# scalable-arch/CAL_22-MPC

Measured on AMD Instinct MI355X. Metric: 64B blocks/s (whole node) + achieved HBM GB/s fraction; ratio bit-exact vs CPU, higher is better.
Workload: dtype u8; 1 GPU; 268435456 random_u32 64 B blocks per GPU, VPC probe config (6 modules, all predictors); algorithm=VPC, line_size=64, blocks_per_gpu=268435456

## Files before the change

cal_22-mpc_amd/csrc/mpc_ring.h:

```cpp
#pragma once
#include "mpc_kernel_common.h"

#ifndef MPC_RING_NT
#define MPC_RING_NT 1
#endif

template <int NQ>
__device__ __forceinline__ u32 ring_swz(u32 line) { return (line >> (NQ == 2 ? 3 : (NQ == 4 ? 2 : 1))) & (u32)(NQ - 1); }

template <int NQ>
__device__ __forceinline__ u32 ring_src_off(int j, u32 lane)
{
  const u32 q = 64u * (u32)j + lane, line = q / NQ, pos = q % NQ;
  return 16u * (line * NQ + (pos ^ ring_swz<NQ>(line))) - 1024u * (u32)j;
}

template <int NQ>
__device__ __forceinline__ u32 ring_rd_off(u32 ll, int k) { return 16u * (ll * NQ + ((u32)k ^ ring_swz<NQ>(ll))); }

#if MPC_RING_NT
#define MPC_GLDS_AUX " nt"
#else
#define MPC_GLDS_AUX ""
#endif
template <int NP>
__device__ __forceinline__ void ring_glds(const u32 *lane_off, const void *gbase, u32 lds_dst)
{
  u32 keep;
  if constexpr (NP == 4)
    asm volatile("s_mov_b32 %0, m0\n\ts_mov_b32 m0, %6\n\ts_nop 0\n\t"
                 "global_load_lds_dwordx4 %1, %5" MPC_GLDS_AUX "\n\tglobal_load_lds_dwordx4 %2, %5 offset:1024" MPC_GLDS_AUX "\n\t"
                 "global_load_lds_dwordx4 %3, %5 offset:2048" MPC_GLDS_AUX "\n\tglobal_load_lds_dwordx4 %4, %5 offset:3072" MPC_GLDS_AUX "\n\t"
                 "s_mov_b32 m0, %0"
                 : "=&s"(keep) : "v"(lane_off[0]), "v"(lane_off[1]), "v"(lane_off[2]), "v"(lane_off[3]), "s"(gbase), "s"(lds_dst));
  else
    asm volatile("s_mov_b32 %0, m0\n\ts_mov_b32 m0, %4\n\ts_nop 0\n\t"
                 "global_load_lds_dwordx4 %1, %3" MPC_GLDS_AUX "\n\tglobal_load_lds_dwordx4 %2, %3 offset:1024" MPC_GLDS_AUX "\n\t"
                 "s_mov_b32 m0, %0"
                 : "=&s"(keep) : "v"(lane_off[0]), "v"(lane_off[1]), "s"(gbase), "s"(lds_dst));
}

template <int NQ>
__device__ __forceinline__ void ring_request(const u32 (&lane_off)[NQ], const uint4 *gbase_, u32 lds_dst_)
{
  const u64 gb = reinterpret_cast<u64>(gbase_);
  const u32 gb_hi = (u32)__builtin_amdgcn_readfirstlane((int)(u32)(gb >> 32)), gb_lo = (u32)__builtin_amdgcn_readfirstlane((int)(u32)gb);
  const uint4 *gbase = reinterpret_cast<const uint4 *>(((u64)gb_hi << 32) | (u64)gb_lo);
  const u32 lds_dst = (u32)__builtin_amdgcn_readfirstlane((int)lds_dst_);
  if constexpr (NQ == 8) {
    ring_glds<4>(&lane_off[0], gbase, lds_dst);
    ring_glds<4>(&lane_off[4], gbase + 256, lds_dst + 4096u);
  } else {
    ring_glds<NQ>(&lane_off[0], gbase, lds_dst);
  }
}

__device__ __forceinline__ u32 uni(u32 x) { return (u32)__builtin_amdgcn_readfirstlane((int)x); }
__device__ __forceinline__ bool uni(bool x) { return __builtin_amdgcn_readfirstlane((int)x) != 0; }

template <int N>
__device__ __forceinline__ void ring_wait_vm() { asm volatile("s_waitcnt vmcnt(%0)" ::"i"(N)); }

template <int NQ>
__device__ __forceinline__ void ring_read(uint4 (&v)[NQ], const u32 (&a)[NQ])
{
  typedef u32 v4 __attribute__((ext_vector_type(4)));
  v4 r[NQ];
  if constexpr (NQ == 2)
    asm volatile("ds_read_b128 %0, %2\n\tds_read_b128 %1, %3\n\ts_waitcnt lgkmcnt(0)"
                 : "=&v"(r[0]), "=&v"(r[1]) : "v"(a[0]), "v"(a[1]));
  else if constexpr (NQ == 4)
    asm volatile("ds_read_b128 %0, %4\n\tds_read_b128 %1, %5\n\tds_read_b128 %2, %6\n\tds_read_b128 %3, %7\n\ts_waitcnt lgkmcnt(0)"
                 : "=&v"(r[0]), "=&v"(r[1]), "=&v"(r[2]), "=&v"(r[3]) : "v"(a[0]), "v"(a[1]), "v"(a[2]), "v"(a[3]));
  else
    asm volatile("ds_read_b128 %0, %8\n\tds_read_b128 %1, %9\n\tds_read_b128 %2, %10\n\tds_read_b128 %3, %11\n\t"
                 "ds_read_b128 %4, %12\n\tds_read_b128 %5, %13\n\tds_read_b128 %6, %14\n\tds_read_b128 %7, %15\n\ts_waitcnt lgkmcnt(0)"
                 : "=&v"(r[0]), "=&v"(r[1]), "=&v"(r[2]), "=&v"(r[3]), "=&v"(r[4]), "=&v"(r[5]), "=&v"(r[6]), "=&v"(r[7])
                 : "v"(a[0]), "v"(a[1]), "v"(a[2]), "v"(a[3]), "v"(a[4]), "v"(a[5]), "v"(a[6]), "v"(a[7]));
#pragma unroll
  for (int k = 0; k < NQ; k++) v[k] = make_uint4(r[k].x, r[k].y, r[k].z, r[k].w);
}
```

cal_22-mpc_amd/csrc/mpc_vpc_lane.hip:

```cpp
#include "mpc_kernel_common.h"
#include "mpc_ring.h"

#ifndef MPC_JIT_BM
#define MPC_JIT_BM 0
#endif
#ifndef MPC_JIT_ANYROOT
#define MPC_JIT_ANYROOT 0
#endif
#ifndef MPC_JIT_PLANES
#define MPC_JIT_PLANES 0
#endif
#ifndef MPC_JIT_GATHER
#define MPC_JIT_GATHER 0
#endif
#ifndef MPC_JIT_WSHIFT
#define MPC_JIT_WSHIFT 0
#endif
#ifndef MPC_DRAIN_WAIT
#define MPC_DRAIN_WAIT 1
#endif
#ifndef MPC_CERT_TIERS
#define MPC_CERT_TIERS 1
#endif
#ifndef MPC_ABLATE
#define MPC_ABLATE 0
#endif
namespace {

constexpr int LK_PW = 8;
constexpr int LK_PW2 = 16;
__device__ __host__ constexpr int lk_base(int kind) { return kind & 7; }
__device__ __host__ constexpr int lk_dist(int kind) { return (kind & LK_PW2) ? 2 : ((kind & LK_PW) ? 1 : 0); }

typedef const u32 __attribute__((address_space(4))) *ctab_t;
__device__ __forceinline__ ctab_t lane_tab(const MpcVpcParams &P) { return (ctab_t)(u64)P.tab; }

#if MPC_JIT_ANYROOT || MPC_JIT_GATHER || MPC_JIT_WSHIFT
template <int Q>
__device__ __forceinline__ MpcFastModule lane_fm_const(const MpcVpcParams &P)
{
  MpcFastModule f = P.fm[Q];
#if MPC_JIT_ANYROOT
  constexpr int roots[] = {MPC_JIT_ROOTS};
  f.root = roots[Q];
#endif
#if MPC_JIT_GATHER
  constexpr int gathers[] = {MPC_JIT_GATHERS};
  f.gather = gathers[Q] ? Q + 1 : 0;
#endif
#if MPC_JIT_WSHIFT
  constexpr int wgens[] = {MPC_JIT_WGENS};
  f.wgen = wgens[Q] ? Q + 1 : 0;
#endif
  return f;
}
#define LANE_FM(Q) lane_fm_const<Q>(P)
#else
#define LANE_FM(Q) P.fm[Q]
#endif

template <int W>
struct Lane {
  u32 x[W];
  u32 b0;
  u32 rootb;
  bool gen;
  ctab_t trunc;
};

template <int W>
__device__ __forceinline__ u32 lane_root_bytes(const Lane<W> &c, int root)
{
  const int rw = root >> 2;
  u32 xw = 0;
#pragma unroll
  for (int e = 0; e < (MPC_JIT_ANYROOT ? W : 4); e++) xw = and_or(c.x[e], 0u - (u32)(e == rw), xw);
  return perm(xw, xw, 0x01010101u * (u32)(root & 3));
}
__device__ __forceinline__ u32 lane_onebase_pred(u32 rb, int root, int e)
{
  const u32 here = (e == (root >> 2)) ? (0xffu << (8 * (root & 3))) : 0u;
  return rb & ~here;
}
__device__ __forceinline__ u32 lane_row0_word(u32 msbs, int root, int e)
{
  return (MPC_JIT_ANYROOT && e == 3 && root > 15) ? (msbs & 0x00ffffffu) : msbs;
}
template <int W, int NR>
__device__ __forceinline__ void lane_root_to_front(const Lane<W> &c, int root, u32 (&r)[W])
{
  u32 prev = lane_root_bytes<W>(c, root) & 0xff000000u;
#pragma unroll
  for (int e = 0; e < (MPC_JIT_ANYROOT ? NR : (NR < 4 ? NR : 4)); e++) {
    const u32 sh = alignbyte(r[e], prev, 3);
    const int nb = root + 1 - 4 * e;
    const u32 m = nb >= 4 ? ~0u : (nb <= 0 ? 0u : ((1u << (8 * nb)) - 1u));
    prev = r[e];
    r[e] = mask_sel(m, sh, r[e]);
  }
}

__device__ __forceinline__ u32 msb_of_bsub(u32 a, u32 b) { return ((a | H80) - (b & L7F)) ^ a ^ ~b; }

template <int W>
__device__ __forceinline__ u32 plane_bytes(const u32 (&x)[W], int q, int k)
// ... 152 lines not shown
    if (MPC_JIT_ANYROOT && c.gen && E0 == 0 && fm.root > 15) m |= lane_root_bytes<W>(c, fm.root);
  }
  return m & H80;
}

template <int W>
__device__ __forceinline__ u32 lane_leading_zero_rows(const u32 (&r)[W], ctab_t scan_mask = nullptr, u32 plane_mask = ~0u)
{
  constexpr int NG = W / 4;
  u32 S[NG], G = 0;
  if (scan_mask) {
#pragma unroll
    for (int j = 0; j < NG; j++) {
      S[j] = (r[4 * j] & scan_mask[4 * j]) | (r[4 * j + 1] & scan_mask[4 * j + 1]) | (r[4 * j + 2] & scan_mask[4 * j + 2]) |
             (r[4 * j + 3] & scan_mask[4 * j + 3]);
      G |= S[j];
    }
  } else {
#pragma unroll
    for (int j = 0; j < NG; j++) {
      S[j] = r[4 * j] | r[4 * j + 1] | r[4 * j + 2] | r[4 * j + 3];
      G |= S[j];
    }
  }
  const u32 gf = fold8(G) & plane_mask;
  const u32 p = (u32)__clz((int)gf) - 24u;
  const u32 B = H80 >> (p & 7u);
  u32 j_star = NG - 1;
#pragma unroll
  for (int j = NG - 2; j >= 0; j--) j_star = (S[j] & B) ? (u32)j : j_star;
  return (plane_mask == ~0u ? G : gf) ? NG * p + j_star : 2u * W;
}

__device__ __forceinline__ bool lane_bit(u64 mask) { return __builtin_amdgcn_inverse_ballot_w64(mask); }

template <int W>
struct LaneBest {
  u32 r[W];
  u32 z;
  int q;
  u32 root_r;
  u32 cx;
  u32 pm;
  u32 encb;
};

#ifndef MPC_DEFER_MAX
#define MPC_DEFER_MAX 8
#endif

#ifndef MPC_PAIR_PROBE
#define MPC_PAIR_PROBE 64
#endif
constexpr u32 kPairProbe = MPC_PAIR_PROBE;

__host__ __device__ static inline size_t lane_stats_smem(int K, int bins)
{
  return 16 * (size_t)((2 * K * 8 + 15) / 16) + 16 * (size_t)(((K * bins + 2) * 4 + 15) / 16);
}

template <int W, int KIND>
__device__ __forceinline__ u32 lane_row0_bm(const Lane<W> &c, const MpcFastModule &fm, ctab_t tab)
{
  u32 r[W], root_r;
  lane_residue<W, KIND, 1>(c, fm, tab, r, root_r);
  return r[0] & (c.trunc ? (c.trunc[0] & 0xffffu) : 0xffffu);
}

template <int W, int NPT, int Q>
__device__ __forceinline__ u32 lane_row0_min(const Lane<W> &, const MpcVpcParams &) { return ~0u; }

template <int W, int NPT, int Q, int KIND, int... REST>
__device__ __forceinline__ u32 lane_row0_min(const Lane<W> &c, const MpcVpcParams &P)
{
  if constexpr (Q + 1 == NPT) {
    return ~0u;
  } else {
    const u32 m = MPC_JIT_BM ? lane_row0_bm<W, KIND>(c, LANE_FM(Q), lane_tab(P)) : lane_row0<W, KIND, 0, 3>(c, LANE_FM(Q), lane_tab(P));
    return min(m, lane_row0_min<W, NPT, Q + 1, REST...>(c, P));
  }
}

template <int W, int NPT, int Q>
__device__ __forceinline__ u32 lane_prefilters(const Lane<W> &, const MpcVpcParams &, u64 &, u64 &, bool, bool &) { return 0; }

template <int W, int NPT, int Q, int KIND, int... REST>
__device__ __forceinline__ u32 lane_prefilters(const Lane<W> &c, const MpcVpcParams &P, u64 &need_mask, u64 &defer_mask,
                                               bool allow_defer, bool &alt)
{
  if constexpr (Q + 1 == NPT) {
    return 0;
  } else {
    u32 bit = 0;
    if constexpr (!(MPC_ABLATE & 8)) {
      u32 msb = MPC_JIT_BM ? lane_row0_bm<W, KIND>(c, LANE_FM(Q), lane_tab(P)) : lane_row0<W, KIND, 0, 3>(c, LANE_FM(Q), lane_tab(P));
      if ((__ballot(msb != 0) & need_mask) != need_mask) {
        if (!MPC_JIT_BM) msb |= lane_row0<W, KIND, 3, 4>(c, LANE_FM(Q), lane_tab(P));
        const u64 pass = ~__ballot(msb != 0) & need_mask;
        if (pass) {
          if (MPC_DEFER_MAX > 0 && W <= 16 && allow_defer && __popcll(pass) <= MPC_DEFER_MAX) {
            defer_mask |= pass;
            need_mask &= ~pass;
          } else {
            bit = 1u << Q;
            const u64 even = 0x5555555555555555ull;
            if (__popcll(pass) >= 16 && ((pass & even) == 0 || (pass & ~even) == 0) &&
                __popcll(need_mask & ~pass) >= 16)
              alt = true;
          }
        }
      }
    }
    return bit | lane_prefilters<W, NPT, Q + 1, REST...>(c, P, need_mask, defer_mask, allow_defer, alt);
  }
}

template <int W, int NR>
__device__ __forceinline__ u32 lane_leading_zero_rows_bm(const u32 (&r)[W], ctab_t scan_mask, u32 none);

template <int W, int NPT, int Q>
__device__ __forceinline__ void lane_seq(const Lane<W> &, const MpcVpcParams &, u32, LaneBest<W> &, bool) {}

template <int W, int NPT, int Q, int KIND, int... REST>
__device__ __forceinline__ void lane_seq(const Lane<W> &c, const MpcVpcParams &P, u32 keep_bits, LaneBest<W> &best,
                                         bool any_full)
{
  constexpr bool last = Q + 1 == NPT;
  if (last || (keep_bits & (1u << Q))) {
    u32 r[W], root_r;
    lane_residue<W, KIND>(c, LANE_FM(Q), lane_tab(P), r, root_r);
    if (c.gen && LANE_FM(Q).root != 0) lane_root_to_front<W, W>(c, LANE_FM(Q).root, r);
    const u32 pm_q = MPC_JIT_PLANES ? LANE_FM(Q).plane_mask : (c.gen ? P.plane_mask : ~0u);
    const u32 z = MPC_JIT_BM ? lane_leading_zero_rows_bm<W, W>(r, c.gen ? c.trunc : nullptr, 2u * W)
                             : lane_leading_zero_rows<W>(r, c.gen ? c.trunc : nullptr, pm_q);
    if (!any_full) {
      best.z = z;
      best.q = Q;
      best.root_r = root_r;
      best.cx = (u32)LANE_FM(Q).cx;
      best.pm = pm_q;
      best.encb = (u32)P.enc_bits[P.start + Q + 1];
#pragma unroll
      for (int e = 0; e < W; e++) best.r[e] = r[e];
    } else {
      const u32 m = best.z <= z ? ~0u : 0u;
      best.z = mask_sel(m, z, best.z);
      best.q = (int)mask_sel(m, (u32)Q, (u32)best.q);
      best.root_r = mask_sel(m, root_r, best.root_r);
      best.cx = mask_sel(m, (u32)LANE_FM(Q).cx, best.cx);
      if (MPC_JIT_PLANES) best.pm = mask_sel(m, pm_q, best.pm);
      best.encb = mask_sel(m, (u32)P.enc_bits[P.start + Q + 1], best.encb);
#pragma unroll
      for (int e = 0; e < W; e++) best.r[e] = mask_sel(m, r[e], best.r[e]);
    }
    any_full = true;
  }
  if constexpr (!last) lane_seq<W, NPT, Q + 1, REST...>(c, P, keep_bits, best, any_full);
}

template <int... KINDS>
__device__ __host__ constexpr bool lane_last_has_root_r()
{
  constexpr int n = sizeof...(KINDS);
  constexpr int kinds[n > 0 ? n : 1] = {KINDS...};
  return n > 0 && lk_base(kinds[n > 0 ? n - 1 : 0]) == MPC_FK_CONSEC;
}

template <int W, int NPT, int Q>
__device__ __forceinline__ void lane_last(const Lane<W> &, const MpcVpcParams &, LaneBest<W> &) {}

template <int W, int NPT, int Q, int KIND, int... REST>
__device__ __forceinline__ void lane_last(const Lane<W> &c, const MpcVpcParams &P, LaneBest<W> &best)
{
  if constexpr (Q + 1 == NPT) {
    u32 zero_root_r;
    lane_residue<W, KIND>(c, LANE_FM(Q), lane_tab(P), best.r, lk_base(KIND) == MPC_FK_CONSEC ? best.root_r : zero_root_r);
    if (c.gen && LANE_FM(Q).root != 0) lane_root_to_front<W, W>(c, LANE_FM(Q).root, best.r);
    best.pm = MPC_JIT_PLANES ? LANE_FM(Q).plane_mask : ~0u;
  } else {
    lane_last<W, NPT, Q + 1, REST...>(c, P, best);
  }
}


template <int W, int NR>
__device__ __forceinline__ u32 lane_leading_zero_rows_bm(const u32 (&r)[W], ctab_t scan_mask, u32 none)
{
  u32 fe = NR, fw = 0;
#pragma unroll
  for (int e = NR - 1; e >= 0; e--) {
    const u32 v = scan_mask ? (r[e] & scan_mask[e]) : r[e];
// ... 274 lines not shown
}

__device__ __forceinline__ u32 encode_rows_x4(const u32 *t, u32 &Z)
{
  u32 P[16];
#pragma unroll
  for (int e = 0; e < 4; e++) {
    const u32 lo01 = perm(t[4 + e], t[e], 0x05010400u), hi01 = perm(t[4 + e], t[e], 0x07030602u);
    const u32 lo23 = perm(t[12 + e], t[8 + e], 0x05010400u), hi23 = perm(t[12 + e], t[8 + e], 0x07030602u);
    P[4 * e] = perm(lo23, lo01, 0x05040100u);
    P[4 * e + 1] = perm(lo23, lo01, 0x07060302u);
    P[4 * e + 2] = perm(hi23, hi01, 0x05040100u);
    P[4 * e + 3] = perm(hi23, hi01, 0x07060302u);
  }
  u32 c2[8];
  u32 s0, s1, s2, s3, s4;
#define MPC_FA(S, C, a, b, c) { S = xor3(a, b, c); C = maj3(a, b, c); }
  MPC_FA(s0, c2[0], P[0], P[1], P[2])
  MPC_FA(s1, c2[1], P[3], P[4], P[5])
  MPC_FA(s2, c2[2], P[6], P[7], P[8])
  MPC_FA(s3, c2[3], P[9], P[10], P[11])
  MPC_FA(s4, c2[4], P[12], P[13], P[14])
  u32 s5, s6;
  MPC_FA(s5, c2[5], s0, s1, s2)
  MPC_FA(s6, c2[6], s3, s4, P[15])
  const u32 b0 = s5 ^ s6;
  c2[7] = s5 & s6;
  u32 d0, d1, d2, c4a, c4b, c4c;
  MPC_FA(d0, c4a, c2[0], c2[1], c2[2])
  MPC_FA(d1, c4b, c2[3], c2[4], c2[5])
  MPC_FA(d2, c4c, d0, d1, c2[6])
#undef MPC_FA
  const u32 b1 = d2 ^ c2[7];
  const u32 hi = or3(c4a, c4b, c4c) | (d2 & c2[7]);
  constexpr unsigned ADJ = (BO_A & BO_B) | (BO_B & BO_C);
  const u32 A = or3(or3(bitop3<ADJ>(P[0], P[1], P[2]), bitop3<ADJ>(P[2], P[3], P[4]), bitop3<ADJ>(P[4], P[5], P[6])),
                    or3(bitop3<ADJ>(P[6], P[7], P[8]), bitop3<ADJ>(P[8], P[9], P[10]), bitop3<ADJ>(P[10], P[11], P[12])),
                    and_or(P[14], P[15], bitop3<ADJ>(P[12], P[13], P[14])));
  const u32 Sf = or3(or3(P[0], P[1], P[2]), or3(P[3], P[4], P[5]), P[6] | P[7]);
  const u32 Sb = or3(or3(P[8], P[9], P[10]), or3(P[11], P[12], P[13]), P[14] | P[15]);
  const u32 single = bitop3<(BO_A & ~BO_B & ~BO_C) & 0xFFu>(b0, b1, hi);
  const u32 cnt2 = bitop3<(~BO_A & BO_B & ~BO_C) & 0xFFu>(b0, b1, hi);
  const u32 two = cnt2 & A;
  const u32 rest = bitop3<(BO_A | (BO_B & ~BO_C)) & 0xFFu>(and_or(b0, b1, hi), cnt2, A);
  const u32 half = bitop3<(BO_A & ~(BO_B & BO_C)) & 0xFFu>(rest, Sf, Sb);
  const u32 full = bitop3<(BO_A & BO_B & BO_C)>(rest, Sf, Sb);
  Z = ~(Sf | Sb);
  return 7u * __popc(single) + 8u * __popc(two) + 12u * __popc(half) + 17u * __popc(full);
}

template <int W>
__device__ __forceinline__ u32 lane_encode(const u32 (&t)[W])
{
  constexpr int NG = W / 4;
  u32 bits = 0;
  u64 ZP = 0;
  if constexpr (NG >= 4) {
#pragma unroll
    for (int h = 0; h < NG / 4; h++) {
      u32 Z;
      bits += encode_rows_x4(&t[16 * h], Z);
      ZP |= (u64)Z << (32 * h);
    }
  } else {
#pragma unroll
    for (int j = 0; j < NG; j++) {
      u32 Z;
      bits += encode_rows(&t[4 * j], Z);
      ZP |= (u64)Z << (8 * j);
    }
  }
  constexpr u64 all = NG == 8 ? ~0ull : ((1ull << (8 * (NG & 7))) - 1ull);
  const u64 prevP = ((ZP << 8) & all) | (ZP >> (8 * (NG - 1) + 1));
  const u64 nextP = (ZP >> 8) | ((ZP & 0x7full) << (8 * (NG - 1) + 1));
  const u64 starts = ZP & ~prevP;
  return bits + 4u * (u32)__popcll(starts) + 3u * (u32)__popcll(starts & nextP);
}

struct LaneRun {
  u32 key;
  u32 cnt;
  u32 acc_r, acc_r2;
  bool enc_hot;
};

__device__ __forceinline__ void lane_run_flush(const LaneRun &rs, const WgStats &st, int K, int bins)
{
  if (rs.cnt) {
    const int k = (int)(rs.key >> 16);
    atomicAdd(&st.hist[k * bins + (int)(rs.key & 0xffffu)], rs.cnt);
    if (rs.acc_r | rs.acc_r2) {
      atomicAdd(&st.sums[k], (u64)rs.acc_r);
      atomicAdd(&st.sums[K + k], (u64)rs.acc_r2);
    }
  }
}

struct LaneEnv {
  WgStats st;
  int K, bins;
  u32 enc_zero, enc_same, enc_unc;
  u32 n_lines, lane;
  u64 first_line;
  uint16_t *sizes_out;
  int8_t *sel_out;
  u32 *defer_q;
  u32 defer_cap;
  u64 *routes;
};

template <int W>
__device__ __forceinline__ void byte_sums(const u32 (&w)[W], u32 &sum, u32 &sum2)
{
  u32 a0 = 0, a1 = 0, q0 = 0, q1 = 0;
#pragma unroll
  for (int e = 0; e < W; e += 2) {
    a0 = sum_bytes(w[e], a0);
    q0 = sum_sq_bytes(w[e], q0);
    a1 = sum_bytes(w[e + 1], a1);
    q1 = sum_sq_bytes(w[e + 1], q1);
  }
  sum = a0 + a1;
  sum2 = q0 + q1;
}

__device__ __forceinline__ void lane_run_add(LaneRun &rs, u32 key, u32 sum_r, u32 sum_r2, const LaneEnv &E)
{
  if (key != rs.key) {
    lane_run_flush(rs, E.st, E.K, E.bins);
    rs.key = key;
    rs.cnt = 0;
    rs.acc_r = 0;
    rs.acc_r2 = 0;
  }
  rs.cnt++;
  rs.acc_r += sum_r;
  rs.acc_r2 += sum_r2;
}

template <int W, bool OUT, bool GEN, bool FULL, bool DRAIN, int... KINDS>
__device__ __forceinline__ void lane_step(const uint4 (&v)[W / 4], u32 line0, u32 loff, u32 dline, bool dvalid,
                                          const MpcVpcParams &P, const LaneEnv &E, LaneRun &rs, u32 &qn, bool &alt)
{
  constexpr int L = 4 * W;
  constexpr int NQ = W / 4;
  constexpr int NPT = sizeof...(KINDS);
  constexpr u32 uncomp = 8u * L;
  const u32 line = DRAIN ? dline : line0 + loff;
  const bool valid = DRAIN ? dvalid : (FULL ? true : (line < E.n_lines));
  const u64 valid_mask = (FULL && !DRAIN) ? ~0ull : __ballot(valid);
  Lane<W> c;
  c.gen = GEN;
#pragma unroll
  for (int i = 0; i < NQ; i++) {
    c.x[4 * i] = v[i].x; c.x[4 * i + 1] = v[i].y; c.x[4 * i + 2] = v[i].z; c.x[4 * i + 3] = v[i].w;
  }

  u64 zero_mask = 0, rep_mask = 0;
  if (__ballot(valid && c.x[1] == c.x[0])) {
    u32 diff = 0;
#pragma unroll
    for (int e = 1; e < W; e++) diff |= c.x[e] ^ c.x[0];
    rep_mask = __ballot(valid && diff == 0);
    zero_mask = __ballot(valid && (diff | c.x[0]) == 0);
  }
  u64 need_mask = valid_mask & ~(zero_mask | (P.has_aws ? rep_mask : 0ull));
  u64 defer_mask = 0;

  u32 sum_r = 0, sum_r2 = 0;
  int n_chosen;
  u32 n_size;
  bool all_unc = false;
  u32 key = 0;

  ctab_t scan_mask = ((NPT == 0 || (GEN && P.plane_mask == ~0u)) && P.trunc_off >= 0) ? lane_tab(P) + P.trunc_off : nullptr;
  c.trunc = GEN ? scan_mask : nullptr;
  if (need_mask) {
    c.b0 = c.x[0] & 0xffu;
    c.rootb = perm(c.x[0], c.x[0], 0u);
    LaneBest<W> best;
    u32 keep_bits = 0;
    if constexpr (NPT > 0) {
      const bool allow_defer = !DRAIN && E.defer_cap != 0u && qn + (u32)((NPT - 1) * MPC_DEFER_MAX) <= E.defer_cap;
      if ((__ballot(lane_row0_min<W, NPT, 0, KINDS...>(c, P) != 0u) & need_mask) != need_mask)
        keep_bits = lane_prefilters<W, NPT, 0, KINDS...>(c, P, need_mask, defer_mask, allow_defer, alt);
      if (!DRAIN && defer_mask) {
        const u32 rank = __builtin_amdgcn_mbcnt_hi((u32)(defer_mask >> 32), __builtin_amdgcn_mbcnt_lo((u32)defer_mask, 0u));
        if (lane_bit(defer_mask)) E.defer_q[qn + rank] = line;
        qn += (u32)__popcll(defer_mask);
      }
      if (keep_bits == 0) lane_last<W, NPT, 0, KINDS...>(c, P, best);
      else lane_seq<W, NPT, 0, KINDS...>(c, P, keep_bits, best, false);
    } else {
      lane_seq_runtime<W>(c, P, best, scan_mask, need_mask);
    }
    u32 kb = keep_bits;
    asm volatile("" : "+s"(kb));
    const bool last_only = NPT > 0 && kb == 0;
    u32 last_cx = 0;
    if constexpr (NPT > 0) last_cx = (u32)LANE_FM(NPT - 1).cx;
    const bool no_pred = NPT == 0 && P.n_pred == 0;
    const u32 unc_size = (no_pred ? 0u : uncomp) + E.enc_unc;

    u32 t[W];
    const u32 best_root_r = (last_only && !lane_last_has_root_r<KINDS...>()) ? 0u : best.root_r;
    const u64 cx_mask = last_only ? (last_cx ? ~0ull : 0ull) : __ballot(best.cx != 0);
    if ((cx_mask & need_mask) == need_mask) {
#pragma unroll
      for (int e = 0; e < W; e++) t[e] = best.r[e] ^ ((best.r[e] >> 1) & (e == 0 ? 0x7f7f7f00u : L7F));
    } else {
      const u32 bcx = last_only ? last_cx : best.cx;
      const u32 cx7 = bcx ? L7F : 0u, ncx = bcx ? 0u : ~0u;
#pragma unroll
      for (int e = 0; e < W; e++) {
        const u32 a = best.r[e] & H80;
        const u32 f = ((best.r[e] >> 1) & cx7) | ((a - (a >> 7)) & ncx);
        t[e] = best.r[e] ^ (e == 0 ? (f & 0xffffff00u) : f);
      }
    }
    if ((NPT == 0 || GEN) && scan_mask) {
#pragma unroll
      for (int e = 0; e < W; e++) t[e] &= scan_mask[e];
    }
    if (MPC_JIT_PLANES && NPT > 0) {
#pragma unroll
      for (int e = 0; e < W; e++) t[e] &= best.pm;
    }
    if (GEN && P.plane_mask != ~0u) {
#pragma unroll
      for (int e = 0; e < W; e++) t[e] &= P.plane_mask;
    }
    u64 open_mask = need_mask;
    const bool byte_major = (NPT == 0 && P.byte_major) || (MPC_JIT_BM && NPT > 0);
    if constexpr (MPC_CERT_TIERS && W == 16 && NPT > 0 && !GEN && !MPC_JIT_BM) {
      if (!rs.enc_hot) {
        LaneFolds<W> folds;
        lane_folds<W>(t, folds);
        open_mask &= ~lane_certified_fast<W>(folds);
        if (MPC_TESTING && E.lane == 0) route_add(E.routes, MPC_RT_VPC_CERT_GROUPS, 1u);
        if (__builtin_expect(open_mask != 0, 0)) {
          open_mask &= ~__ballot(lane_certified_exact<W>(t, folds));
          if (MPC_TESTING && E.lane == 0) route_add(E.routes, MPC_RT_VPC_CERT_EXACT, 1u);
        }
      }
    } else {
      if (!rs.enc_hot && !byte_major) open_mask &= ~__ballot(lane_certified<W>(t));
    }
    if (MPC_JIT_BM && NPT > 0 && !rs.enc_hot) open_mask &= ~__ballot(lane_certified_bm<W>(t));
    if constexpr (MPC_ABLATE & 16) {
      if (open_mask) E.st.hist[0] = 1u;
      open_mask = 0;
    }
    u32 enc = uncomp;
    u64 keep_mask = 0;
    if (open_mask) {
      if (MPC_TESTING && E.lane == 0) route_add(E.routes, MPC_RT_VPC_ENCODER, 1u);
      if (byte_major) enc = lane_encode_bm<W>(t);
      else enc = lane_encode<W>(t);
      if (!no_pred) keep_mask = __ballot(enc < uncomp) & open_mask;
    }
    rs.enc_hot = keep_mask != 0;

    if (keep_mask == 0 && need_mask == valid_mask) {
      if constexpr (MPC_ABLATE & 4) { sum_r = c.x[3]; sum_r2 = c.x[5]; }
      else byte_sums<W>(c.x, sum_r, sum_r2);
      all_unc = true;
      key = unc_size;
      if constexpr (OUT) {
        if (valid) {
          const u64 at = E.first_line + line;
          if (E.sizes_out) E.sizes_out[at] = (uint16_t)unc_size;
          if (E.sel_out) E.sel_out[at] = (int8_t)-1;
        }
      }
    } else {
      const bool keep = lane_bit(keep_mask);
      if (keep_mask == need_mask) {
        const u32 w0 = mask_sel(0xffu, best_root_r, best.r[0]);
        u32 a0 = sum_bytes(w0, 0u), q0 = sum_sq_bytes(w0, 0u), a1 = 0, q1 = 0;
#pragma unroll
        for (int e = 1; e < W; e += 2) {
          a1 = sum_bytes(best.r[e], a1);
          q1 = sum_sq_bytes(best.r[e], q1);
          if (e + 1 < W) {
            a0 = sum_bytes(best.r[e + 1], a0);
            q0 = sum_sq_bytes(best.r[e + 1], q0);
          }
        }
        sum_r = a0 + a1;
        sum_r2 = q0 + q1;
      } else {
        u32 w[W];
        const u32 km = keep ? ~0u : 0u;
#pragma unroll
        for (int e = 0; e < W; e++) w[e] = mask_sel(km, best.r[e], c.x[e]);
        w[0] = mask_sel(km & 0xffu, best_root_r, w[0]);
        byte_sums<W>(w, sum_r, sum_r2);
      }
      const bool need = lane_bit(need_mask);
      sum_r = need ? sum_r : 0u;
      sum_r2 = need ? sum_r2 : 0u;
      if (keep_mask) {
        u32 last_encb = 0;
        if constexpr (NPT > 0) last_encb = (u32)P.enc_bits[P.start + NPT];
        n_chosen = keep ? P.start + (last_only ? NPT - 1 : best.q) : -1;
        n_size = keep ? enc + (last_only ? last_encb : best.encb) : unc_size;
      } else {
        n_chosen = -1;
        n_size = unc_size;
      }
    }
  }

  if (!all_unc) {
    const bool is_zero = lane_bit(zero_mask), need = lane_bit(need_mask), deferred = !DRAIN && lane_bit(defer_mask);
    const int chosen = need ? n_chosen : (is_zero ? 0 : 1);
    const u32 size = need ? n_size : (is_zero ? E.enc_zero : E.enc_same);
    key = ((u32)(chosen + 1) << 16) | size;
    if (!DRAIN) key = deferred ? ((u32)E.K << 16) : key;

    if constexpr (OUT) {
      if (valid && !deferred) {
        const u64 at = E.first_line + line;
        if (E.sizes_out) E.sizes_out[at] = (uint16_t)size;
        if (E.sel_out) E.sel_out[at] = (int8_t)chosen;
      }
    }
  }

  if (FULL && !DRAIN && __ballot(key != rs.key) == 0) {
    rs.cnt++;
    rs.acc_r += sum_r;
    rs.acc_r2 += sum_r2;
  } else if (valid) {
    lane_run_add(rs, key, sum_r, sum_r2, E);
  }
}

constexpr int kWaitVm0 = (7 << 4) | (15 << 8);

template <int NQ>
__device__ __forceinline__ void lane_fetch(uint4 (&v)[NQ], const uint4 *__restrict__ lines, u32 line, u32 n_lines)
{
  const uint4 *src = lines + (u64)min(line, n_lines - 1u) * NQ;
#pragma unroll
  for (int i = 0; i < NQ; i++) v[i] = src[i];
}

#ifndef MPC_LANE_WAVES
#define MPC_LANE_WAVES 16
#endif
#ifndef MPC_LANE_WAVES_128
#define MPC_LANE_WAVES_128 8
#endif
#ifndef MPC_LANE_WAVES_32
#define MPC_LANE_WAVES_32 16
#endif
__host__ __device__ constexpr int lane_wpb_of(int L) { return L <= 32 ? MPC_LANE_WAVES_32 : (L <= 64 ? MPC_LANE_WAVES : MPC_LANE_WAVES_128); }
template <int W, int NPT>
__host__ __device__ constexpr int lane_wpb() { return NPT == 0 ? 4 : lane_wpb_of(4 * W); }

struct LaneLds {
  u32 stages;
  u32 cap;
  size_t bytes;
};
__host__ __device__ static inline size_t lane_ring_off(size_t stats_and_queues) { return (stats_and_queues + 1023u) & ~(size_t)1023u; }

static LaneLds lane_lds_plan(const MpcVpcParams *P, int wpb, bool wants_queue)
{
  const size_t stats = lane_stats_smem(P->M + 1, P->hist_bins), SB = 64u * (size_t)P->L, lds = 160u << 10;
  const u32 caps[5] = {wants_queue ? 256u : 0u, wants_queue ? 192u : 0u, wants_queue ? 160u : 0u, wants_queue ? 96u : 0u, 0u};
  for (u32 cap : caps) {
    const size_t bytes = lane_ring_off(stats + (size_t)wpb * cap * sizeof(u32)) + (size_t)wpb * 2u * SB;
    if (bytes <= lds) return LaneLds{2, cap, bytes};
  }
  return LaneLds{0, 0, 0};
}

#ifndef MPC_LB_WAVES
#define MPC_LB_WAVES 4
#endif
#ifndef MPC_LB_WAVES_RT
#define MPC_LB_WAVES_RT 3
#endif
#ifndef MPC_LB_WAVES_128
#define MPC_LB_WAVES_128 2
#endif
template <int W, bool OUT, bool GEN, int... KINDS>
__device__ __forceinline__ void vpc_lane_body(unsigned char *smem, const uint4 *__restrict__ lines, u32 n_lines, u64 first_line,
                                              const MpcVpcParams &P, uint16_t *__restrict__ sizes_out, int8_t *__restrict__ sel_out,
                                              u64 *gstats, u32 ring_cfg)
{
  constexpr int NQ = W / 4;
  constexpr u32 WPB = lane_wpb<W, sizeof...(KINDS)>();
  LaneEnv E;
  E.K = P.M + 1;
  E.bins = P.hist_bins;
  E.st.sums = reinterpret_cast<u64 *>(smem);
  E.st.hist = reinterpret_cast<u32 *>(smem + 16 * ((2 * E.K * 8 + 15) / 16));
  if (threadIdx.x == 0) E.st.hist[E.K * E.bins + 1] = 0;
  stats_init(E.st, E.K, E.bins, threadIdx.x, 64 * (int)WPB);
  E.defer_cap = ring_cfg >> 8;
  E.defer_q = reinterpret_cast<u32 *>(smem + lane_stats_smem(E.K, E.bins)) + (threadIdx.x >> 6) * E.defer_cap;
  E.enc_zero = (u32)P.enc_bits[1];
  E.enc_same = 32u + (u32)P.enc_bits[2];
  E.enc_unc = (u32)P.enc_bits[0];
  E.n_lines = n_lines;
  E.lane = threadIdx.x & 63;
  E.first_line = first_line;
  E.sizes_out = sizes_out;
  E.sel_out = sel_out;

  LaneRun rs = {0xffffffffu, 0, 0, 0, false};
  u32 iter = 0;
  const u32 wave = __builtin_amdgcn_readfirstlane(threadIdx.x >> 6);
  u64 *routes = gstats + (2 * E.K + E.K * E.bins);
  E.routes = MPC_TESTING ? routes : nullptr;
#if MPC_STAMPS
  u64 *stamp = routes + MPC_ROUTE_COUNT + 3u * blockIdx.x;
  if (sizeof...(KINDS) > 0 && threadIdx.x == 0 && blockIdx.x < (u32)MPC_STAMP_WGS) {
    stamp[0] = wall_clock64();
    stamp[2] = ((u64)__builtin_amdgcn_s_getreg((31 << 11) | 20) << 32) | (u64)__builtin_amdgcn_s_getreg((31 << 11) | 4);
  }
#endif
  bool alt = false;
  uint4 va[NQ];
  u32 qn = 0;
  if constexpr (sizeof...(KINDS) == 0) {
    uint4 vb[NQ];
    const u32 stride = gridDim.x * WPB * 64u;
    u32 line0 = (blockIdx.x * WPB + wave) * 64u;
    if (line0 < n_lines) lane_fetch<NQ>(va, lines, line0 + E.lane, n_lines);
    while (line0 < n_lines) {
      lane_fetch<NQ>(vb, lines, line0 + stride + E.lane, n_lines);
      lane_step<W, OUT, false, false, false>(va, line0, E.lane, 0u, true, P, E, rs, qn, alt);
      line0 += stride;
#pragma unroll
      for (int i = 0; i < NQ; i++) va[i] = vb[i];
      if ((++iter & 255u) == 0) {
        lane_run_flush(rs, E.st, E.K, E.bins);
        rs.cnt = 0;
        rs.acc_r = 0;
        rs.acc_r2 = 0;
      }
    }
  } else {
    constexpr u32 SB = 64u * 4u * W;
    constexpr u32 kNone = 0xffffffffu;
    const u32 defer_high = E.defer_cap >= 64u ? E.defer_cap - 64u : 0u;
    const u32 ring_lds = (u32)lane_ring_off(lane_stats_smem(E.K, E.bins) + WPB * E.defer_cap * sizeof(u32)) + wave * (2u * SB);
    u32 lane_off[NQ];
#pragma unroll
    for (int j = 0; j < NQ; j++) lane_off[j] = ring_src_off<NQ>(j, E.lane);
    const u32 rd0 = (ring_lds + 16u * NQ * E.lane) | (16u * ring_swz<NQ>(E.lane));
    const u32 n_blocks = n_lines >> 7;
    const u32 per_wg = uni((n_blocks + gridDim.x - 1u) / gridDim.x);
    const u32 b_begin = blockIdx.x * per_wg;
    const u32 b_end = b_begin + per_wg < n_blocks ? b_begin + per_wg : n_blocks;
    u32 *ticket = E.st.hist + E.K * E.bins + 1;
    auto claim = [&]() -> u32 {
      u32 t = 0;
      if (E.lane == 0) t = atomicAdd(ticket, 1u);
      const u32 blk = b_begin + uni(t);
      return uni((b_begin < n_blocks && blk < b_end) ? blk : kNone);
    };
    auto request = [&](u32 blk, u32 h) { ring_request<NQ>(lane_off, lines + (u64)(2u * blk + h) * (64u * NQ), ring_lds + h * SB); };
    u32 cb = claim();
    if (cb != kNone) {
      request(cb, 0u);
      request(cb, 1u);
    }
    u32 paired = 0;
    u32 pair_left = 0;
    bool tail_done = false;
    for (;;) {
      while (cb != kNone && qn <= defer_high) {
        cb = uni(cb);
        qn = uni(qn);
        iter = uni(iter);
        const u32 pair_now = uni(paired);
        const u32 nb = claim();
        for (u32 h = 0; h < 2u; h = uni(h + 1u)) {
          u32 a0;
          if (pair_now) {
            ring_wait_vm<0>();
            const u32 bl = 2u * E.lane + h;
            a0 = (ring_lds + 16u * NQ * bl) | (16u * ring_swz<NQ>(bl & 63u));
          } else {
            if (h == 0u || nb != kNone) ring_wait_vm<NQ>();
            else ring_wait_vm<0>();
            a0 = rd0 + h * SB;
          }
          u32 a[NQ];
#pragma unroll
          for (int j = 0; j < NQ; j++) a[j] = a0 ^ (16u * (u32)j);
          ring_read<NQ>(va, a);
          if constexpr (!(MPC_ABLATE & 32)) {
            if (nb != kNone) {
              if (!pair_now) {
                request(nb, h);
              } else if (h == 1u) {
                request(nb, 0u);
                request(nb, 1u);
              }
            }
          }
          __builtin_amdgcn_sched_barrier(0);
          lane_step<W, OUT, GEN, true, false, KINDS...>(va, pair_now ? cb * 128u + h : cb * 128u + h * 64u, pair_now ? 2u * E.lane : E.lane,
                                                   0u, true, P, E, rs, qn, alt);
          if ((++iter & 255u) == 0) {
            lane_run_flush(rs, E.st, E.K, E.bins);
            rs.cnt = 0;
            rs.acc_r = 0;
            rs.acc_r2 = 0;
          }
        }
        alt = uni(alt);
        paired = uni(paired);
        pair_left = uni(pair_left);
        if (MPC_TESTING && E.lane == 0) route_add(routes, pair_now ? MPC_RT_VPC_PAIRED_BLOCKS : MPC_RT_VPC_PLAIN_BLOCKS, 1u);
        if (paired) {
          if (--pair_left == 0u) {
            paired = 0u;
            if (MPC_TESTING && E.lane == 0) route_add(routes, MPC_RT_VPC_TO_PLAIN, 1u);
          }
        } else if (alt) {
          paired = 1u;
          pair_left = kPairProbe;
          if (MPC_TESTING && E.lane == 0) route_add(routes, MPC_RT_VPC_TO_PAIRED, 1u);
        }
        alt = false;
        cb = nb;
      }
      const bool tail_mine = !tail_done && cb == kNone && blockIdx.x == gridDim.x - 1u && wave == 0u;
      u32 tail_l0 = n_blocks * 128u;
      for (;;) {
        u32 dline;
        bool dvalid;
        if (qn > 0u) {
          const u32 take = qn < 64u ? qn : 64u;
          qn -= take;
          if (MPC_TESTING && E.lane == 0) {
            route_add(routes, MPC_RT_VPC_DRAINS, 1u);
            route_add(routes, MPC_RT_VPC_DEFERRED, take);
          }
          dvalid = E.lane < take;
          dline = dvalid ? E.defer_q[qn + E.lane] : 0u;
        } else if (tail_mine && tail_l0 < n_lines) {
          dline = tail_l0 + E.lane;
          dvalid = dline < n_lines;
          tail_l0 += 64u;
          if (MPC_TESTING && E.lane == 0) route_add(routes, MPC_RT_VPC_TAIL_GROUPS, 1u);
        } else {
          break;
        }
        lane_fetch<NQ>(va, lines, dline, n_lines);
        if constexpr (MPC_DRAIN_WAIT) __builtin_amdgcn_s_waitcnt(kWaitVm0);
        lane_step<W, OUT, GEN, false, true, KINDS...>(va, 0u, 0u, dline, dvalid, P, E, rs, qn, alt);
      }
      if (tail_mine) tail_done = true;
      if (cb == kNone && (tail_done || blockIdx.x != gridDim.x - 1u || wave != 0u)) break;
    }
  }
  lane_run_flush(rs, E.st, E.K, E.bins);
  stats_flush(E.st, E.K, E.bins, gstats, (int)(E.lane + 64u * wave), 64 * (int)WPB);
#if MPC_STAMPS
  if (sizeof...(KINDS) > 0 && E.lane + 64u * wave == 0u && blockIdx.x < (u32)MPC_STAMP_WGS) stamp[1] = wall_clock64();
#endif
}

#define MPC_LANE_BOUNDS(W, NPT)                                                                                     \
  __launch_bounds__((64 * lane_wpb<W, NPT>()),                                                                      \
                    (W <= 16 ? (NPT > 0 ? (W == 8 && MPC_LANE_WAVES_32 == 10 ? 5 : MPC_LB_WAVES) : MPC_LB_WAVES_RT) : MPC_LB_WAVES_128))
template <int W, bool OUT, int... KINDS>
__global__ void MPC_LANE_BOUNDS(W, (sizeof...(KINDS)))
vpc_lane_kernel(const uint4 *__restrict__ lines, u32 n_lines, u64 first_line, MpcVpcParams P,
                uint16_t *__restrict__ sizes_out, int8_t *__restrict__ sel_out, u64 *gstats, u32 ring_cfg)
{
  extern __shared__ __attribute__((aligned(16))) unsigned char smem[];
  vpc_lane_body<W, OUT, false, KINDS...>(smem, lines, n_lines, first_line, P, sizes_out, sel_out, gstats, ring_cfg);
}
template <int W, bool OUT, int... KINDS>
__global__ void MPC_LANE_BOUNDS(W, (sizeof...(KINDS)))
vpc_lane_gen_kernel(const uint4 *__restrict__ lines, u32 n_lines, u64 first_line, MpcVpcParams P,
                    uint16_t *__restrict__ sizes_out, int8_t *__restrict__ sel_out, u64 *gstats, u32 ring_cfg)
{
  extern __shared__ __attribute__((aligned(16))) unsigned char smem[];
  vpc_lane_body<W, OUT, true, KINDS...>(smem, lines, n_lines, first_line, P, sizes_out, sel_out, gstats, ring_cfg);
}

#ifndef MPC_LANE_JIT
#define OB MPC_FK_ONEBASE
#define CS MPC_FK_CONSEC
#define DF MPC_FK_DIFF
#define WT MPC_FK_WEIGHT

template <int... KINDS>
bool lane_seq_matches(const MpcVpcParams *P)
{
  constexpr int n = sizeof...(KINDS);
  const int kinds[n > 0 ? n : 1] = {KINDS...};
  if (P->n_pred != n || n == 0 || P->runtime_only) return false;
  for (int q = 0; q < n; q++) {
    const MpcFastModule &f = P->fm[q];
    if (f.kind != lk_base(kinds[q])) return false;
    if (lk_dist(kinds[q]) ? f.prev_word != lk_dist(kinds[q]) : f.prev_word == 2) return false;
  }
  return true;
}

template <int... KINDS>
hipError_t lane_launch(const uint4 *l, u32 n_lines, u64 first_line, const MpcVpcParams *P, uint16_t *d_sizes,
                       int8_t *d_sel, u64 *d_stats, int grid, hipStream_t stream)
{
#define MPC_LAUNCH_K(KERNEL, WV, OUTV)                                                                               \
  {                                                                                                                \
    if (smem > (64u << 10))                                                                                        \
      (void)hipFuncSetAttribute(reinterpret_cast<const void *>(&KERNEL<WV, OUTV, KINDS...>),                       \
                                hipFuncAttributeMaxDynamicSharedMemorySize, (int)smem);                            \
    hipLaunchKernelGGL((KERNEL<WV, OUTV, KINDS...>), dim3(wgrid), dim3(64 * wpb), smem, stream, l, n_lines,         \
                       first_line, *P, d_sizes, d_sel, d_stats, ring_cfg);                                         \
  }
#define MPC_LAUNCH(WV)                                                                                              \
  {                                                                                                                \
    constexpr int wpb = lane_wpb<WV, sizeof...(KINDS)>();                                                          \
    size_t smem;                                                                                                   \
    u32 ring_cfg = 0;                                                                                              \
    int wgrid;                                                                                                     \
    if (sizeof...(KINDS) == 0) {                                                                                   \
      smem = lane_stats_smem(P->M + 1, P->hist_bins);                                                              \
      wgrid = grid;                                                                                                \
    } else {                                                                                                       \
      const LaneLds plan = lane_lds_plan(P, wpb, WV <= 16);                                                        \
      if (plan.stages == 0) return hipErrorInvalidConfiguration;              \
      smem = plan.bytes;                                                                                           \
      ring_cfg = plan.stages | (plan.cap << 8);                                                                    \
           \
                 \
      const u64 want = (n_lines / 64u + (u64)wpb - 1u) / (u64)wpb;                                                 \
      const u64 cap = (u64)grid / (wpb == 16 ? 16u : 8u);        \
      wgrid = (int)(want < cap ? want : cap);                                                                      \
      if (wgrid < 1) wgrid = 1;                                                                                    \
    }                                                                                                              \
    const bool out = d_sizes || d_sel;                                                                             \
    bool gen_done = false;                                                                                         \
    if constexpr (sizeof...(KINDS) > 0) {                                                                          \
// ... 177 lines not shown
```

Before: 103.4 billion blocks/s.

## Add uncompressible-run fast path and immediate-offset LDS ring reads

Adds a per-lane 'urun' counter so that consecutive all-uncompressed blocks in the full ring path skip the ballot, key comparison and run bookkeeping, accumulating byte sums directly into the running stats and folding the deferred count at flush and run boundaries. Separately, ring reads in the unpaired path now use precomputed per-slot LDS addresses with a compile-time ds_read_b128 offset, which removes per-iteration address arithmetic. Bool flags become u32 to help keep them in scalar or uniform registers. The change adds more state to the run-tracking logic, and a mistake in counting the deferred run would break the statistics.

```diff
diff --git a/cal_22-mpc_amd/csrc/mpc_ring.h b/cal_22-mpc_amd/csrc/mpc_ring.h
--- a/cal_22-mpc_amd/csrc/mpc_ring.h
+++ b/cal_22-mpc_amd/csrc/mpc_ring.h
@@ -61,22 +61,25 @@
 template <int N>
 __device__ __forceinline__ void ring_wait_vm() { asm volatile("s_waitcnt vmcnt(%0)" ::"i"(N)); }
 
-template <int NQ>
+template <int NQ, u32 OFF = 0>
 __device__ __forceinline__ void ring_read(uint4 (&v)[NQ], const u32 (&a)[NQ])
 {
+  static_assert(OFF < 65536u, "ds_read_b128: the offset field has 16 bits");
   typedef u32 v4 __attribute__((ext_vector_type(4)));
   v4 r[NQ];
   if constexpr (NQ == 2)
-    asm volatile("ds_read_b128 %0, %2\n\tds_read_b128 %1, %3\n\ts_waitcnt lgkmcnt(0)"
-                 : "=&v"(r[0]), "=&v"(r[1]) : "v"(a[0]), "v"(a[1]));
+    asm volatile("ds_read_b128 %0, %2 offset:%4\n\tds_read_b128 %1, %3 offset:%4\n\ts_waitcnt lgkmcnt(0)"
+                 : "=&v"(r[0]), "=&v"(r[1]) : "v"(a[0]), "v"(a[1]), "i"(OFF));
   else if constexpr (NQ == 4)
-    asm volatile("ds_read_b128 %0, %4\n\tds_read_b128 %1, %5\n\tds_read_b128 %2, %6\n\tds_read_b128 %3, %7\n\ts_waitcnt lgkmcnt(0)"
-                 : "=&v"(r[0]), "=&v"(r[1]), "=&v"(r[2]), "=&v"(r[3]) : "v"(a[0]), "v"(a[1]), "v"(a[2]), "v"(a[3]));
+    asm volatile("ds_read_b128 %0, %4 offset:%8\n\tds_read_b128 %1, %5 offset:%8\n\tds_read_b128 %2, %6 offset:%8\n\t"
+                 "ds_read_b128 %3, %7 offset:%8\n\ts_waitcnt lgkmcnt(0)"
+                 : "=&v"(r[0]), "=&v"(r[1]), "=&v"(r[2]), "=&v"(r[3]) : "v"(a[0]), "v"(a[1]), "v"(a[2]), "v"(a[3]), "i"(OFF));
   else
-    asm volatile("ds_read_b128 %0, %8\n\tds_read_b128 %1, %9\n\tds_read_b128 %2, %10\n\tds_read_b128 %3, %11\n\t"
-                 "ds_read_b128 %4, %12\n\tds_read_b128 %5, %13\n\tds_read_b128 %6, %14\n\tds_read_b128 %7, %15\n\ts_waitcnt lgkmcnt(0)"
+    asm volatile("ds_read_b128 %0, %8 offset:%16\n\tds_read_b128 %1, %9 offset:%16\n\tds_read_b128 %2, %10 offset:%16\n\t"
+                 "ds_read_b128 %3, %11 offset:%16\n\tds_read_b128 %4, %12 offset:%16\n\tds_read_b128 %5, %13 offset:%16\n\t"
+                 "ds_read_b128 %6, %14 offset:%16\n\tds_read_b128 %7, %15 offset:%16\n\ts_waitcnt lgkmcnt(0)"
                  : "=&v"(r[0]), "=&v"(r[1]), "=&v"(r[2]), "=&v"(r[3]), "=&v"(r[4]), "=&v"(r[5]), "=&v"(r[6]), "=&v"(r[7])
-                 : "v"(a[0]), "v"(a[1]), "v"(a[2]), "v"(a[3]), "v"(a[4]), "v"(a[5]), "v"(a[6]), "v"(a[7]));
+                 : "v"(a[0]), "v"(a[1]), "v"(a[2]), "v"(a[3]), "v"(a[4]), "v"(a[5]), "v"(a[6]), "v"(a[7]), "i"(OFF));
 #pragma unroll
   for (int k = 0; k < NQ; k++) v[k] = make_uint4(r[k].x, r[k].y, r[k].z, r[k].w);
 }
diff --git a/cal_22-mpc_amd/csrc/mpc_vpc_lane.hip b/cal_22-mpc_amd/csrc/mpc_vpc_lane.hip
--- a/cal_22-mpc_amd/csrc/mpc_vpc_lane.hip
+++ b/cal_22-mpc_amd/csrc/mpc_vpc_lane.hip
@@ -21,6 +21,9 @@
 #endif
 #ifndef MPC_CERT_TIERS
 #define MPC_CERT_TIERS 1
+#endif
+#ifndef MPC_RING_OFS
+#define MPC_RING_OFS 1
 #endif
 #ifndef MPC_ABLATE
 #define MPC_ABLATE 0
@@ -339,11 +342,11 @@
 }
 
 template <int W, int NPT, int Q>
-__device__ __forceinline__ u32 lane_prefilters(const Lane<W> &, const MpcVpcParams &, u64 &, u64 &, bool, bool &) { return 0; }
+__device__ __forceinline__ u32 lane_prefilters(const Lane<W> &, const MpcVpcParams &, u64 &, u64 &, bool, u32 &) { return 0; }
 
 template <int W, int NPT, int Q, int KIND, int... REST>
 __device__ __forceinline__ u32 lane_prefilters(const Lane<W> &c, const MpcVpcParams &P, u64 &need_mask, u64 &defer_mask,
-                                               bool allow_defer, bool &alt)
+                                               bool allow_defer, u32 &alt)
 {
   if constexpr (Q + 1 == NPT) {
     return 0;
@@ -363,7 +366,7 @@
             const u64 even = 0x5555555555555555ull;
             if (__popcll(pass) >= 16 && ((pass & even) == 0 || (pass & ~even) == 0) &&
                 __popcll(need_mask & ~pass) >= 16)
-              alt = true;
+              alt = 1u;
           }
         }
       }
@@ -804,7 +807,22 @@
   u32 cnt;
   u32 acc_r, acc_r2;
   bool enc_hot;
+  u32 urun;
 };
+
+__device__ __forceinline__ void lane_run_fold(LaneRun &rs)
+{
+  if (rs.urun) {
+    rs.cnt += rs.urun - 1u;
+    rs.urun = 1u;
+  }
+}
+__device__ __forceinline__ u32 lane_run_leave(LaneRun &rs)
+{
+  const u32 more = rs.urun > 1u ? rs.urun : 1u;
+  rs.urun = 0u;
+  return more;
+}
 
 __device__ __forceinline__ void lane_run_flush(const LaneRun &rs, const WgStats &st, int K, int bins)
 {
@@ -845,6 +863,20 @@
   sum = a0 + a1;
   sum2 = q0 + q1;
 }
+template <int W>
+__device__ __forceinline__ void byte_sums_into(const u32 (&w)[W], u32 &acc, u32 &acc2)
+{
+  u32 a0 = acc, a1 = 0, q0 = acc2, q1 = 0;
+#pragma unroll
+  for (int e = 0; e < W; e += 2) {
+    a0 = sum_bytes(w[e], a0);
+    q0 = sum_sq_bytes(w[e], q0);
+    a1 = sum_bytes(w[e + 1], a1);
+    q1 = sum_sq_bytes(w[e + 1], q1);
+  }
+  acc = a0 + a1;
+  acc2 = q0 + q1;
+}
 
 __device__ __forceinline__ void lane_run_add(LaneRun &rs, u32 key, u32 sum_r, u32 sum_r2, const LaneEnv &E)
 {
@@ -862,7 +894,7 @@
 
 template <int W, bool OUT, bool GEN, bool FULL, bool DRAIN, int... KINDS>
 __device__ __forceinline__ void lane_step(const uint4 (&v)[W / 4], u32 line0, u32 loff, u32 dline, bool dvalid,
-                                          const MpcVpcParams &P, const LaneEnv &E, LaneRun &rs, u32 &qn, bool &alt)
+                                          const MpcVpcParams &P, const LaneEnv &E, LaneRun &rs, u32 &qn, u32 &alt)
 {
   constexpr int L = 4 * W;
   constexpr int NQ = W / 4;
@@ -892,7 +924,7 @@
   u32 sum_r = 0, sum_r2 = 0;
   int n_chosen;
   u32 n_size;
-  bool all_unc = false;
+  u32 all_unc = 0;
   u32 key = 0;
 
   ctab_t scan_mask = ((NPT == 0 || (GEN && P.plane_mask == ~0u)) && P.trunc_off >= 0) ? lane_tab(P) + P.trunc_off : nullptr;
@@ -984,9 +1016,20 @@
     rs.enc_hot = keep_mask != 0;
 
     if (keep_mask == 0 && need_mask == valid_mask) {
+      if (FULL && !DRAIN && rs.urun != 0u) {
+        if constexpr (MPC_ABLATE & 4) { rs.acc_r += c.x[3]; rs.acc_r2 += c.x[5]; }
+        else byte_sums_into<W>(c.x, rs.acc_r, rs.acc_r2);
+        rs.urun++;
+        if constexpr (OUT) {
+          const u64 at = E.first_line + line;
+          if (E.sizes_out) E.sizes_out[at] = (uint16_t)unc_size;
+          if (E.sel_out) E.sel_out[at] = (int8_t)-1;
+        }
+        return;
+      }
       if constexpr (MPC_ABLATE & 4) { sum_r = c.x[3]; sum_r2 = c.x[5]; }
       else byte_sums<W>(c.x, sum_r, sum_r2);
-      all_unc = true;
+      all_unc = 1u;
       key = unc_size;
       if constexpr (OUT) {
         if (valid) {
@@ -1050,12 +1093,15 @@
     }
   }
 
+  const u32 more = lane_run_leave(rs);
   if (FULL && !DRAIN && __ballot(key != rs.key) == 0) {
-    rs.cnt++;
+    rs.cnt += more;
     rs.acc_r += sum_r;
     rs.acc_r2 += sum_r2;
-  } else if (valid) {
-    lane_run_add(rs, key, sum_r, sum_r2, E);
+    rs.urun = all_unc;
+  } else {
+    rs.cnt += more - 1u;
+    if (valid) lane_run_add(rs, key, sum_r, sum_r2, E);
   }
 }
 
@@ -1134,7 +1180,7 @@
   E.sizes_out = sizes_out;
   E.sel_out = sel_out;
 
-  LaneRun rs = {0xffffffffu, 0, 0, 0, false};
+  LaneRun rs = {0xffffffffu, 0, 0, 0, false, 0};
   u32 iter = 0;
   const u32 wave = __builtin_amdgcn_readfirstlane(threadIdx.x >> 6);
   u64 *routes = gstats + (2 * E.K + E.K * E.bins);
@@ -1146,7 +1192,7 @@
     stamp[2] = ((u64)__builtin_amdgcn_s_getreg((31 << 11) | 20) << 32) | (u64)__builtin_amdgcn_s_getreg((31 << 11) | 4);
   }
 #endif
-  bool alt = false;
+  u32 alt = 0;
   uint4 va[NQ];
   u32 qn = 0;
   if constexpr (sizeof...(KINDS) == 0) {
@@ -1176,6 +1222,9 @@
 #pragma unroll
     for (int j = 0; j < NQ; j++) lane_off[j] = ring_src_off<NQ>(j, E.lane);
     const u32 rd0 = (ring_lds + 16u * NQ * E.lane) | (16u * ring_swz<NQ>(E.lane));
+    u32 rd[NQ];
+#pragma unroll
+    for (int j = 0; j < NQ; j++) rd[j] = rd0 ^ (16u * (u32)j);
     const u32 n_blocks = n_lines >> 7;
     const u32 per_wg = uni((n_blocks + gridDim.x - 1u) / gridDim.x);
     const u32 b_begin = blockIdx.x * per_wg;
@@ -1204,20 +1253,33 @@
         const u32 pair_now = uni(paired);
         const u32 nb = claim();
         for (u32 h = 0; h < 2u; h = uni(h + 1u)) {
-          u32 a0;
-          if (pair_now) {
-            ring_wait_vm<0>();
-            const u32 bl = 2u * E.lane + h;
-            a0 = (ring_lds + 16u * NQ * bl) | (16u * ring_swz<NQ>(bl & 63u));
+          if (pair_now || !MPC_RING_OFS) {
+            u32 a0;
+            if (pair_now) {
+              ring_wait_vm<0>();
+              const u32 bl = 2u * E.lane + h;
+              a0 = (ring_lds + 16u * NQ * bl) | (16u * ring_swz<NQ>(bl & 63u));
+            } else {
+              if (h == 0u || nb != kNone) ring_wait_vm<NQ>();
+              else ring_wait_vm<0>();
+              a0 = rd0 + h * SB;
+            }
+            u32 a[NQ];
+#pragma unroll
+            for (int j = 0; j < NQ; j++) a[j] = a0 ^ (16u * (u32)j);
+            ring_read<NQ>(va, a);
           } else {
-            if (h == 0u || nb != kNone) ring_wait_vm<NQ>();
-            else ring_wait_vm<0>();
-            a0 = rd0 + h * SB;
+            if (h == 0u) {
+              ring_wait_vm<NQ>();
+              ring_read<NQ, 0u>(va, rd);
+            } else if (nb != kNone) {
+              ring_wait_vm<NQ>();
+              ring_read<NQ, SB>(va, rd);
+            } else {
+              ring_wait_vm<0>();
+              ring_read<NQ, SB>(va, rd);
+            }
           }
-          u32 a[NQ];
-#pragma unroll
-          for (int j = 0; j < NQ; j++) a[j] = a0 ^ (16u * (u32)j);
-          ring_read<NQ>(va, a);
           if constexpr (!(MPC_ABLATE & 32)) {
             if (nb != kNone) {
               if (!pair_now) {
@@ -1232,6 +1294,7 @@
           lane_step<W, OUT, GEN, true, false, KINDS...>(va, pair_now ? cb * 128u + h : cb * 128u + h * 64u, pair_now ? 2u * E.lane : E.lane,
                                                    0u, true, P, E, rs, qn, alt);
           if ((++iter & 255u) == 0) {
+            lane_run_fold(rs);
             lane_run_flush(rs, E.st, E.K, E.bins);
             rs.cnt = 0;
             rs.acc_r = 0;
@@ -1252,7 +1315,7 @@
           pair_left = kPairProbe;
           if (MPC_TESTING && E.lane == 0) route_add(routes, MPC_RT_VPC_TO_PAIRED, 1u);
         }
-        alt = false;
+        alt = 0u;
         cb = nb;
       }
       const bool tail_mine = !tail_done && cb == kNone && blockIdx.x == gridDim.x - 1u && wave == 0u;
@@ -1285,6 +1348,7 @@
       if (cb == kNone && (tail_done || blockIdx.x != gridDim.x - 1u || wave != 0u)) break;
     }
   }
+  lane_run_fold(rs);
   lane_run_flush(rs, E.st, E.K, E.bins);
   stats_flush(E.st, E.K, E.bins, gstats, (int)(E.lane + 64u * wave), 64 * (int)WPB);
 #if MPC_STAMPS
```

New measurement: 104.2 billion blocks/s, median of 6. About the same (+0.8%).
